# benattal/neural-radiance-caching

Measured on AMD Instinct MI355X. Metric: rays/sec (1024-ray batch, 64+64 proposal + 32 shaded samples/ray), hotdog cache forward, higher is better.
Workload: dtype f32

## Files before the change

neural-radiance-caching_amd/csrc/hostcheck.cpp:

```cpp
#include <stdio.h>
#include <stdlib.h>

#include <string>

#include "rc_pack_host.h"
#include "rc_ide_coef.h"
#include "rc_vis_plan.h"
#include "rc_ws.h"

using namespace rcpack;

static std::vector<float> read_f32(const std::string& path, size_t count) {
  std::vector<float> v(count);
  FILE* f = fopen(path.c_str(), "rb");
  if (!f || fread(v.data(), sizeof(float), count, f) != count) { fprintf(stderr, "hostcheck: cannot read %zu floats from %s\n", count, path.c_str()); exit(2); }
  fclose(f);
  return v;
}
static void write_f32(const std::string& path, const std::vector<float>& v) {
  FILE* f = fopen(path.c_str(), "wb");
  if (!f || fwrite(v.data(), sizeof(float), v.size(), f) != v.size()) { fprintf(stderr, "hostcheck: cannot write %s\n", path.c_str()); exit(2); }
  fclose(f);
}
static HostLayer layer(const std::string& dir, const char* name, int in, int out) {
// ... 23 lines not shown

static int transient_heads(const std::string& dir) {
  HostLayer slf = layer(dir, "slf", 128, 71), irr = layer(dir, "irr", 64, 70);
  write_f32(dir + "/out_tbins_split.bin", pack_bins_stream(slf, irr, 70, 192, true));
  write_f32(dir + "/out_tbins_f32.bin", pack_bins_stream(slf, irr, 70, 128, false));
  write_f32(dir + "/out_tslice_slf.bin", pack_slice_columns(slf, 4, 70, 132));
  write_f32(dir + "/out_tslice_irr.bin", pack_slice_columns(irr, 2, 70, 68));
  std::vector<float> v;
  for (float sigma : {3.0f, 4.0f, 0.7f, 0.0f}) {
    const std::vector<float> t = temporal_taps(sigma);
    v.push_back((float)t.size());
    v.insert(v.end(), t.begin(), t.end());
  }
  write_f32(dir + "/out_ttaps.bin", v);
  printf("hostcheck tbins ok\n");
  return 0;
}

template <size_t... K> static void emplace_kind(WsExtra& x, size_t kind, std::index_sequence<K...>) {
  ((kind == K ? (void)x.emplace<K>() : (void)0), ...);
}
static long ws_offset(WsBufs& s, const WsBuf* b) { return (long)((const char*)b - (const char*)&s); }
static int ws_registry(int num_levels, int n_names, char** names) {
  std::vector<WsBufs> sets(WS_COUNT);
  long lookups = 0;
  for (int id = 0; id < WS_COUNT; ++id) emplace_kind(sets[id].x, kWsSets[id].kind, std::make_index_sequence<std::variant_size_v<WsExtra>>());
  for (int id = 0; id < WS_COUNT; ++id) {
    WsBufs& s = sets[id];
    if (s.x.index() != kWsSets[id].kind) return 5;
    for (const WsName& e : wsn::kTable)
// ... 12 lines not shown
  for (int i = 0; i < n_names; ++i) {
    std::string leaf;
    const int id = ws_split(names[i], leaf);
    const WsBuf* b = id < 0 ? nullptr : ws_lookup(sets[id], leaf, num_levels);
    ++lookups;
    if (b) printf("probe %s %d %ld\n", names[i], id, ws_offset(sets[id], b));
    else printf("probe %s %d -\n", names[i], id);
  }
  size_t bufs = 0;
  for (int id = 0; id < WS_COUNT; ++id) ws_for_each(sets[id], [&](WsBuf& b) { bufs += b.p == nullptr; });
  printf("lookups %ld buffers %zu\nhostcheck ws ok\n", lookups, bufs);
  return 0;
}

int main(int argc, char** argv) {
  if (argc < 2) { fprintf(stderr, "usage: hostcheck <dir> | hostcheck --tbins <dir> | hostcheck --ide-inc | hostcheck --ws <num_levels> [name ...]\n"); return 2; }
  if (std::string(argv[1]) == "--ide-inc") return print_ide_inc();
  if (std::string(argv[1]) == "--tbins") {
    if (argc < 3) { fprintf(stderr, "usage: hostcheck --tbins <dir>\n"); return 2; }
    return transient_heads(argv[2]);
  }
  if (std::string(argv[1]) == "--ws") {
    if (argc < 3) { fprintf(stderr, "usage: hostcheck --ws <num_levels> [name ...]\n"); return 2; }
    return ws_registry(atoi(argv[2]), argc - 3, argv + 3);
  }
  const std::string dir = argv[1];
  {
    HostLayer L = layer(dir, "a", 37, 70);
    std::vector<Step> s;
    steps_natural(s, 37, 0); step_bias(s);
    write_f32(dir + "/out_pack.bin", pack(s, {tile_full(&L, 0), tile_full(&L, 1), tile_full(&L, 2)}));
  }
  {
    HostLayer L = layer(dir, "b", 64, 40);
    std::vector<Step> s;
// ... 88 lines not shown
```

neural-radiance-caching_amd/csrc/rc_api.hip:

```cpp
#include <dlfcn.h>
#include <math.h>
#include <stdlib.h>
#include <stdio.h>
#include <string.h>

#include <array>
#include <map>
#include <memory>
#include <string>
#include <variant>
#include <vector>

#include "rc_internal.h"
#include "rc_pack_host.h"
#include "rc_itof_host.h"
#include "rc_ws.h"
#include "rc_prng_host.h"

void rc_launch_hashgrid_src(const RcGridDev& g, const float* points, int soa_in, const int32_t* src, int64_t n_src,
                            int64_t n, float* out, int feature_major, int64_t ldo, float contract_radius,
                            float* jac_out, hipStream_t stream);
int rc_shader_lds_bytes();
int rc_weight_chunk_floats();
void rc_shader_prepare();
// ... 399 lines not shown
    if (hipStreamCreateWithPriority(&s, hipStreamNonBlocking, which == 0 ? prio_lo : prio_hi) != hipSuccess) s = nullptr;
  }
  return s;
}

int ensure_side_stream(rc_handle* h) {
  if (h->side_stream) return RC_OK;
  h->side_stream = rc_helper_stream(0);
  if (!h->side_stream) return fail(h, RC_ERR_HIP, "side stream");
  for (hipEvent_t& e : h->ev_side) RC_HIP(h, hipEventCreateWithFlags(&e, hipEventDisableTiming));
  return RC_OK;
}

int repack_transient(rc_handle* h);

int repack(rc_handle* h) {
  std::string missing;
  const rc_config& c = h->cfg;
  std::vector<float> fused_parts[4];
  if (!h->ide_table.p) {
    RcIdeTable tb;
    build_ide_table(tb);
    RC_HIP(h, hipMalloc((void**)&h->ide_table.p, sizeof(tb)));
    h->ide_table.bytes = sizeof(tb);
    RC_HIP(h, hipMemcpy(h->ide_table.p, &tb, sizeof(tb), hipMemcpyHostToDevice));
  }
  for (int g = 0; g < 4; ++g)
    for (size_t l = 0; l < h->grids[g].sizes.size(); ++l)
      if (!h->grids[g].loaded[l])
        return fail(h, RC_ERR_MISSING_WEIGHT,
                    "missing weight: " + h->grids[g].prefix + "/" + level_name(h->grids[g].cfg, h->grids[g].sizes, h->grids[g].sizes[l]));
  for (int l = 0; l < c.num_levels; ++l) {
    const std::string base = "params/Cache/Sampler/MLP_" + std::to_string(l);
    const HostLayer* d0 = need(h, base + "/density_layers_0", missing);
    const HostLayer* d1 = need(h, base + "/density_layers_1", missing);
    const HostLayer* dout = need(h, base + "/output_density_layer", missing);
    const HostLayer* dn = (l == c.num_levels - 1) ? need(h, base + "/pred_normals_layer", missing) : nullptr;
    if (!missing.empty()) return fail(h, RC_ERR_MISSING_WEIGHT, "missing weight: " + missing);
    std::vector<Step> s;
    steps_natural(s, d0->in, 0); step_bias(s);
    std::vector<float> stream = pack_f32(s, {tile_full(d0, 0), tile_full(d0, 1)});
    s.clear(); steps_acc(s, 2, 0); step_bias(s);
    append(stream, pack_f32(s, {tile_full(d1, 0), tile_full(d1, 1)}));
    std::vector<Col> regs = {Col{dout, 0}};
    if (dn) { regs.push_back(Col{dn, 0}); regs.push_back(Col{dn, 1}); regs.push_back(Col{dn, 2}); }
    append(stream, pack_dot(regs, 2, false));
    if (dn) {
      HostLayer w1t, w0t;
      w1t.in = d1->out; w1t.out = d1->in; w1t.kernel.resize(d1->kernel.size()); w1t.bias.assign(w1t.out, 0.0f);
      for (int r = 0; r < d1->in; ++r) for (int c2 = 0; c2 < d1->out; ++c2) w1t.kernel[(size_t)c2 * w1t.out + r] = d1->kernel[(size_t)r * d1->out + c2];
      w0t.in = d0->out; w0t.out = d0->in; w0t.kernel.resize(d0->kernel.size()); w0t.bias.assign(w0t.out, 0.0f);
      for (int r = 0; r < d0->in; ++r) for (int c2 = 0; c2 < d0->out; ++c2) w0t.kernel[(size_t)c2 * w0t.out + r] = d0->kernel[(size_t)r * d0->out + c2];
      std::vector<Step> sb; steps_acc(sb, 2, 0);
      append(stream, pack_f32(sb, {tile_full(&w1t, 0, 0, false), tile_full(&w1t, 1, 0, false)}));
      append(stream, pack_f32(sb, {tile_full(&w0t, 0, 0, false)}));
    }
    if (l < 3) fused_parts[l] = stream;
    int rc = upload(h, h->packs.dens[l], pad_stream(stream));
    if (rc) return rc;
  }
  if (h->transient) {
    int off[4];
    rc_fused_stream_offsets(&off[0], &off[1], &off[2], &off[3]);
    bool ok = fused_geometry_ok(h);
    std::vector<float> stream;
    for (int p = 0; p < 3 && ok; ++p) {
      ok = (int)(stream.size() / 64) == off[p];
      append(stream, fused_parts[p]);
    }
    if (ok && (int)(stream.size() / 64) < off[3] && off[3] - (int)(stream.size() / 64) < 4) stream.resize((size_t)off[3] * 64, 0.0f);
    ok = ok && (int)(stream.size() / 64) == off[3];
    h->fused_front_ok = ok;
    if (ok) {
      int rc = upload(h, h->packs.fused_front, pad_stream(stream));
      if (rc) return rc;
      if ((rc = build_fused_tables(h))) return rc;
    }
    return repack_transient(h);
  }
  const std::string sh = "params/Cache/Shader";
  const HostLayer* bott = need(h, sh + "/bottleneck_layer", missing);
  const HostLayer* rough = need(h, sh + "/roughness_layer", missing);
  const HostLayer* tint = need(h, sh + "/tint_layer", missing);
  const HostLayer* amb = need(h, sh + "/ambient_irradiance_layer", missing);
  const HostLayer* irr = need(h, sh + "/irradiance_layer", missing);
  const HostLayer* i0 = need(h, sh + "/integrated_brdf_layers_0", missing);
// ... 16 lines not shown
    for (int o = 0; o < lb->out; ++o) lbf.bias[o] = (float)((double)lbf.bias[o] + (double)lb->bias[o]);
    for (int o = 0; o < i0->out; ++o) i0f.bias[o] = (float)((double)i0f.bias[o] + (double)i0->bias[o]);
    steps_acc(s, 2, 0); steps_natural(s, 32, 64); step_bias(s);
    std::vector<Col> regs = {Col{rough, 0}, Col{tint, 0}, Col{tint, 1}, Col{tint, 2}, Col{amb, 0},
                             Col{amb, 1},   Col{amb, 2},  Col{irr, 0},  Col{irr, 1},  Col{irr, 2}};
    append(stream, pack(s, {tile_by_reg(regs)}));
    s.clear(); steps_acc(s, 2, 0); steps_natural(s, 32, 64);
    for (int i = 0; i < 36; ++i) s.push_back({{FE + i, FE + 36 + i}});
    step_bias(s);
    append(stream, pack(s, {tile_full(&l0f, 0), tile_full(&l0f, 1), tile_full(&l0f, 2), tile_full(&l0f, 3),
                            tile_full(&lbf, 0), tile_full(&lbf, 1), tile_full(&lbf, 2), tile_full(&lbf, 3)}));
    s.clear(); steps_acc(s, 2, 0); steps_natural(s, 32, 64); s.push_back({{FE, -2}});
    append(stream, pack(s, {tile_full(&i0f, 0), tile_full(&i0f, 1)}));
    s.clear(); steps_acc(s, 2, 0); step_bias(s);
    append(stream, pack(s, {tile_full(i1, 0), tile_full(i1, 1)}));
    append(stream, pack_dot({Col{io, 0}}, 2));
    s.clear(); steps_acc(s, 4, 0); step_bias(s);
    append(stream, pack(s, {tile_full(l1, 0), tile_full(l1, 1), tile_full(l1, 2), tile_full(l1, 3)}));
    append(stream, pack(s, {tile_full(l2, 0), tile_full(l2, 1), tile_full(l2, 2), tile_full(l2, 3)}));
    std::vector<Step> sb; steps_acc(sb, 4, 0);
    append(stream, pack(sb, {tile_full(lb, 0, 0, false), tile_full(lb, 1, 0, false), tile_full(lb, 2, 0, false),
                             tile_full(lb, 3, 0, false)}));
    append(stream, pack_dot({Col{la, 0}, Col{la, 1}, Col{la, 2}}, 4));
    fused_parts[3] = stream;
    int rc = upload(h, h->packs.shader, pad_stream(stream));
    if (rc) return rc;
  }
  {
    int off[4];
    const int nf = rc_fused_stream_offsets(&off[0], &off[1], &off[2], &off[3]);
    bool ok = fused_geometry_ok(h);
    std::vector<float> stream;
    for (int p = 0; p < 4 && ok; ++p) {
      if (p == 3 && (int)(stream.size() / 64) < off[p] && off[p] - (int)(stream.size() / 64) < 4) stream.resize((size_t)off[p] * 64, 0.0f);
      ok = (int)(stream.size() / 64) == off[p];
      append(stream, fused_parts[p]);
    }
    ok = ok && (int)(stream.size() / 64) == nf;
    h->fused_ok = ok;
    if (ok) {
      int rc = upload(h, h->packs.fused, pad_stream(stream));
      if (rc) return rc;
      if ((rc = build_fused_tables(h))) return rc;
    }
  }
  {
    std::string miss;
    const std::string ep = "params/Cache/EnvMap";
    const HostLayer* e0 = need(h, ep + "/layer_0", miss);
    const HostLayer* e1 = need(h, ep + "/layer_1", miss);
    const HostLayer* e2 = need(h, ep + "/layer_2", miss);
    const HostLayer* eb = need(h, ep + "/layer_bottleneck", miss);
    const HostLayer* eo = need(h, ep + "/output_rgba_layer", miss);
// ... 527 lines not shown
```

neural-radiance-caching_amd/csrc/rc_dev_mlp.h:

```cpp
#pragma once
#include "rc_internal.h"

namespace rcdev {

typedef float f32x16 __attribute__((ext_vector_type(16)));

constexpr int kWaves = 4;

__device__ __forceinline__ f32x16 zero16() {
  f32x16 z;
#pragma unroll
  for (int i = 0; i < 16; ++i) z[i] = 0.0f;
  return z;
}

typedef uint32_t u32x4 __attribute__((ext_vector_type(4)));
typedef __bf16 bf16x8 __attribute__((ext_vector_type(8)));

__device__ __forceinline__ uint32_t pack_top16(float a1, float a0) {
  return __builtin_amdgcn_perm(__float_as_uint(a1), __float_as_uint(a0), 0x07060302u);
}
__device__ __forceinline__ float top16(float a) { return __uint_as_float(__float_as_uint(a) & 0xffff0000u); }
typedef float f32x2 __attribute__((ext_vector_type(2)));
__device__ __forceinline__ f32x2 top16(f32x2 a) { return f32x2{top16(a[0]), top16(a[1])}; }
// ... 410 lines not shown
    for (int p = 0; p < PT; ++p) {
      float sum = part[p][o][0] + part[p][o][1];
      sum = sum + __shfl_xor(sum, 32, 64);
      out[p][o] = sum + bias;
    }
  }
}
template <int NT, int NO, int FBASE, int NF, bool KEEP = false, int W = kWaves, int NOB = NO, int CH = kChunk, class WS = WStream>
__device__ __forceinline__ void dot_out1(const WS& w, const f32x16 (&hid)[NT], float (&out)[NO],
                                         float (&keep)[KEEP ? NT * 16 : 1]) {
  const f32x16 (&h1)[1][NT] = reinterpret_cast<const f32x16 (&)[1][NT]>(hid);
  float (&o1)[1][NO] = reinterpret_cast<float (&)[1][NO]>(out);
  dot_out<1, NT, NO, FBASE, NF, KEEP, W, NOB, CH, WS>(w, h1, o1, keep);
}

__device__ __forceinline__ float softplus(float x) {
  return fmaxf(x, 0.0f) + log1pf(expf(-fabsf(x)));
}
__device__ __forceinline__ float sigmoidf(float x) { return 1.0f / (1.0f + expf(-x)); }
template <class F>
__device__ __forceinline__ void eval_pair(F f, int h, float xa, float xb, float& ya, float& yb) {
  const float y = f(h ? xb : xa);
  ya = y; yb = y;
  swap_halves(ya, yb);
}
__device__ __forceinline__ void softplus_pair(int h, float xa, float xb, float& ya, float& yb) {
  eval_pair([](float x) { return softplus(x); }, h, xa, xb, ya, yb);
}
__device__ __forceinline__ void sigmoid_pair(int h, float xa, float xb, float& ya, float& yb) {
  eval_pair([](float x) { return sigmoidf(x); }, h, xa, xb, ya, yb);
// ... 19 lines not shown
    if (v != v) return 0.0f;
    return fminf(fmaxf(v, -RC_FMAX), RC_FMAX);
  };
  x = fix(nx); y = fix(ny); z = fix(nz);
}


__host__ __device__ constexpr int ide_l(int i) { return i < 2 ? 1 : (i < 5 ? 2 : (i < 10 ? 4 : (i < 19 ? 8 : 16))); }
__host__ __device__ constexpr int ide_m(int i) { return i < 2 ? i : (i < 5 ? i - 2 : (i < 10 ? i - 5 : (i < 19 ? i - 10 : i - 19))); }


constexpr int kShActSteps = 102;
constexpr int kStepIde = 48;
constexpr int kStepBias = 84;

struct ShaderFrags {
  static constexpr int F_H = 0, F_S0 = F_H + rc_lfr(49, 1), F_I0 = F_S0 + rc_lfr(85, 8), F_I1 = F_I0 + rc_lfr(49, 2), F_IO = F_I1 + rc_lfr(33, 2),
                       F_S1 = F_IO + rc_dfr(1, 2), F_S2 = F_S1 + rc_lfr(65, 4), F_SB = F_S2 + rc_lfr(65, 4), F_SO = F_SB + rc_lfr(64, 4),
                       COUNT = F_SO + rc_dfr(3, 4);
};

struct ShaderConsts { float roughness_bias, irradiance_bias, ambient_bias, rgb_max, slf_ambient_bias; };
struct ShadeOut { float rgb[3], ad[3], idf[3], is[3], tint[3]; };

#ifdef RC_STAMPS
#define RC_TSTAMP(i) do { if (st) { __builtin_amdgcn_sched_barrier(0); st[i] = __builtin_amdgcn_s_memtime(); __builtin_amdgcn_sched_barrier(0); } } while (0)
#else
#define RC_TSTAMP(i) do { } while (0)
#endif
template <int F0, int NF, class WS = WStream>
__device__ __forceinline__ ShadeOut shader_tile(const WS& ws, float* act, int lane, int h, float nx, float ny, float nz,
                                                float vx, float vy, float vz, const ShaderConsts& k,
                                                unsigned long long* st = nullptr) {
  RC_TSTAMP(0);
  float rough, tint[3], ad[3], idf[3];
  float tint2_raw, idf2_raw;
  u32x4 fpc[6][3];
  if constexpr (kRcSplit) split_blocks<6>(act, fpc);
  {
    f32x16 acc[1];
    acc[0] = zero16();
    if constexpr (kRcSplit) mlp_layer_x<1, 49, F0 + ShaderFrags::F_H, NF, 6, true>(ws, act, acc, fpc);
    else mlp_layer<1, 49, F0 + ShaderFrags::F_H, NF>(ws, act, acc);
    float sp_ad[3], sp_idf[2];
    softplus_pair(h, acc[0][0] + k.roughness_bias, acc[0][4] + k.ambient_bias, rough, sp_ad[0]);
    softplus_pair(h, acc[0][5] + k.ambient_bias, acc[0][6] + k.ambient_bias, sp_ad[1], sp_ad[2]);
    softplus_pair(h, acc[0][7] + k.irradiance_bias, acc[0][8] + k.irradiance_bias, sp_idf[0], sp_idf[1]);
    sigmoid_pair(h, acc[0][1], acc[0][2], tint[0], tint[1]);
    tint2_raw = acc[0][3];
    idf2_raw = acc[0][9] + k.irradiance_bias;
#pragma unroll
    for (int c = 0; c < 3; ++c) ad[c] = fminf(fmaxf(sp_ad[c], 0.0f), k.rgb_max);
#pragma unroll
    for (int c = 0; c < 2; ++c) idf[c] = fminf(fmaxf(sp_idf[c], 0.0f), k.rgb_max);
  }
  RC_TSTAMP(1);
  float dot_nv;
  {
// ... 21 lines not shown
    for (int i = 0; i < RC_IDE_TERMS; ++i) {
      const int l = ide_l(i), m = ide_m(i);
      float poly = 0.0f;
#pragma unroll
      for (int k = 0; k < RC_IDE_ZPOW; ++k) {
        if (k <= l - m && ((l - m - k) & 1) == 0) poly = poly + zp[k] * kRcIdeCoef[i][k];
      }
      const float att = expf(-(0.5f * (float)(l * (l + 1))) * rough);
      act[(kStepIde + i) * 64] = (cpw[m] * poly) * att;
    }
  }
  RC_TSTAMP(2);
  f32x16 s0[8];
#pragma unroll
  for (int t = 0; t < 8; ++t) s0[t] = zero16();
  if constexpr (kRcSplit) mlp_layer_x<8, 85, F0 + ShaderFrags::F_S0, NF, 6, false>(ws, act, s0, fpc);
  else mlp_layer<8, 85, F0 + ShaderFrags::F_S0, NF>(ws, act, s0);
  RC_TSTAMP(3);
  float ibrdf;
  {
    f32x16 ib[2];
    ib[0] = zero16(); ib[1] = zero16();
    act[48 * 64] = h == 0 ? dot_nv : 1.0f;
    if constexpr (kRcSplit) mlp_layer_x<2, 49, F0 + ShaderFrags::F_I0, NF, 6, false>(ws, act, ib, fpc);
    else mlp_layer<2, 49, F0 + ShaderFrags::F_I0, NF>(ws, act, ib);
    BHand<2, true> hi;
    hand_off<2, true>(ib, lane, hi);
    ib[0] = zero16(); ib[1] = zero16();
    mlp_layer_h<2, 2, true, F0 + ShaderFrags::F_I1, NF>(ws, hi, ib);
    float o[1], nokeep[1];
    dot_out1<2, 1, F0 + ShaderFrags::F_IO, NF>(ws, ib, o, nokeep);
    sigmoid_pair(h, tint2_raw, o[0] + 1.0986123f, tint[2], ibrdf);
  }
  RC_TSTAMP(4);
  float amb[3];
  {
    f32x16 acc[4] = {s0[0], s0[1], s0[2], s0[3]};
    f32x16 skip[4] = {s0[4], s0[5], s0[6], s0[7]};
    BHand<4, true> hs;
    hand_off<4, true>(acc, lane, hs);
#pragma unroll
    for (int t = 0; t < 4; ++t) acc[t] = zero16();
    mlp_layer_h<4, 4, true, F0 + ShaderFrags::F_S1, NF>(ws, hs, acc);
    hand_off<4, true>(acc, lane, hs);
#pragma unroll
    for (int t = 0; t < 4; ++t) acc[t] = zero16();
    RC_TSTAMP(5);
    mlp_layer_h<4, 4, true, F0 + ShaderFrags::F_S2, NF>(ws, hs, acc);
    BHand<4, false> hb;
    hand_off<4, false>(acc, lane, hb);
    RC_TSTAMP(6);
    mlp_layer_h<4, 4, false, F0 + ShaderFrags::F_SB, NF>(ws, hb, skip);
    RC_TSTAMP(7);
    float o[3], nokeep[1];
    dot_out1<4, 3, F0 + ShaderFrags::F_SO, NF>(ws, skip, o, nokeep);
    float sp_idf2, sp_amb[3];
    softplus_pair(h, idf2_raw, o[0] + k.slf_ambient_bias, sp_idf2, sp_amb[0]);
    softplus_pair(h, o[1] + k.slf_ambient_bias, o[2] + k.slf_ambient_bias, sp_amb[1], sp_amb[2]);
    idf[2] = fminf(fmaxf(sp_idf2, 0.0f), k.rgb_max);
#pragma unroll
    for (int c = 0; c < 3; ++c) amb[c] = fmaxf(sp_amb[c], 0.0f);
  }
  RC_TSTAMP(8);
  ShadeOut o;
#pragma unroll
  for (int c = 0; c < 3; ++c) {
    const float is = fminf(fmaxf(tint[c] * ibrdf * (amb[c] * 1.0f), 0.0f), k.rgb_max);
    const float ambient = ad[c] + 0.0f;
    const float indirect = idf[c] + is;
    o.rgb[c] = ambient + indirect; o.ad[c] = ad[c]; o.idf[c] = idf[c]; o.is[c] = is; o.tint[c] = tint[c];
// ... 6 lines not shown
```

neural-radiance-caching_amd/csrc/rc_fused.hip:

```cpp
#include "rc_fused_common.h"
#include <type_traits>

using namespace rcdev;
using namespace rcfused;

namespace {

constexpr int kAppSteps = 32;

#define RC_OUT_PINS "s"(op[0]), "s"(op[1]), "s"(op[2]), "s"(op[3]), "s"(op[4]), "s"(op[5]), "s"(op[6]), "s"(op[7]), "s"(op[8]), "s"(op[9]), \
                    "s"(op[10]), "s"(op[11]), "s"(op[12]), "s"(op[13]), "s"(op[14]), "s"(op[15]), "s"(op[16]), "s"(op[17]), "s"(op[18])
#define RC_EXPORT_PINS "s"(a.f_tdist), "s"(a.f_density), "s"(a.f_means), "s"(a.f_normals_pred), "s"(a.n)

template <int K> struct LookupRegs { const float* table[K]; int32_t size[K]; uint32_t mask[K]; float bbox, precondition, contract_radius, density_bias; };
template <int K>
__device__ __forceinline__ LookupRegs<K> fetch_lookup(const RcLookupRec& q) {
  LookupRegs<K> g;
#pragma unroll
  for (int l = 0; l < K; ++l) { g.table[l] = q.table[l]; g.size[l] = q.size[l]; g.mask[l] = l < kFusedDense ? 0u : q.mask[l]; }
  g.bbox = q.bbox; g.precondition = q.precondition; g.contract_radius = q.contract_radius; g.density_bias = q.density_bias;
  return g;
}
#define RC_LOOKUP_PINS6(g) "s"(g.table[0]), "s"(g.table[1]), "s"(g.table[2]), "s"(g.table[3]), "s"(g.table[4]), "s"(g.table[5]),      \
                           "s"(g.size[0]), "s"(g.size[1]), "s"(g.size[2]), "s"(g.size[3]), "s"(g.size[4]), "s"(g.size[5]),              \
// ... 5 lines not shown
  static_assert(K >= 6 && K <= 8, "RC_LOOKUP_PINS6 and the levels behind it");
  if constexpr (K == 6) asm volatile("" :: RC_LOOKUP_PINS6(g));
  else if constexpr (K == 7) asm volatile("" :: RC_LOOKUP_PINS6(g), "s"(g.table[6]), "s"(g.size[6]), "s"(g.mask[6]));
  else asm volatile("" :: RC_LOOKUP_PINS6(g), "s"(g.table[6]), "s"(g.size[6]), "s"(g.mask[6]), "s"(g.table[7]), "s"(g.size[7]), "s"(g.mask[7]));
}
struct ShadeRegs { ShaderConsts sh; float bg; const float* lights; const float* viewdirs; float pct0, pct1, pct2; };
__device__ __forceinline__ ShadeRegs fetch_shade(const RcShadeRec& q) {
  return ShadeRegs{q.sh, q.bg, q.lights, q.viewdirs, q.pct[0], q.pct[1], q.pct[2]};
}
#define RC_SHADE_PINS(k) "s"(k.sh.roughness_bias), "s"(k.sh.irradiance_bias), "s"(k.sh.ambient_bias), "s"(k.sh.rgb_max), "s"(k.sh.slf_ambient_bias), \
                         "s"(k.bg), "s"(k.lights), "s"(k.viewdirs), "s"(k.pct0), "s"(k.pct1), "s"(k.pct2)

template <int K, int FB, int NF, class WS>
__device__ __forceinline__ float density_level64(const WS& ws, float* act_wave, int lane, const float (&f)[K]) {
  constexpr int KS0 = (K + 1) / 2 + 1;
  using FR = DensFrags<KS0>;
  const int tile = lane >> 5, j = lane & 31, h = lane >> 5;
#pragma unroll
  for (int k = 0; k < 2 * (KS0 - 1); ++k)
    act_wave[tile * kTileStride + (k >> 1) * 64 + j + 32 * (k & 1)] = k < K ? f[k < K ? k : 0] : 0.0f;
#pragma unroll
  for (int p = 0; p < 2; ++p) act_wave[p * kTileStride + (KS0 - 1) * 64 + lane] = h == 0 ? 1.0f : 0.0f;
  lds_sync<false>();
  float* act = act_wave + lane;
  f32x16 acc[2][2];
#pragma unroll
  for (int p = 0; p < 2; ++p) { acc[p][0] = zero16(); acc[p][1] = zero16(); }
  mlp_layer_pt<2, 2, KS0, FB + FR::D0, NF>(ws, act, kTileStride, acc);
  BHandPt<2, 2, true> hd;
#pragma unroll
  for (int p = 0; p < 2; ++p) hand_off<2, true>(acc[p], lane, hd.hand[p]);
#pragma unroll
  for (int p = 0; p < 2; ++p) { acc[p][0] = zero16(); acc[p][1] = zero16(); }
  mlp_layer_pth<2, 2, 2, true, FB + FR::D1, NF>(ws, hd, acc);
  float out[2][1], nokeep[1];
  dot_out<2, 2, 1, FB + FR::DO, NF>(ws, acc, out, nokeep);
  return tile == 0 ? out[0][0] : out[1][0];
}

template <int LEVEL, int K, int FB, int NF, class WS, class FETCH, class PIN>
__device__ __forceinline__ float proposal_level(const LookupRegs<K>& g, const WS& ws, float* act_wave, const Ray& r, const float* s_td, int lane,
                                                unsigned long long* stamps, const FETCH& fetch_next, const PIN& pin_next) {
  float mx, my, mz, t0, t1;
  mean_of(r, s_td, lane, mx, my, mz, t0, t1);
  float cx = mx, cy = my, cz = mz;
  contract3(cx, cy, cz, g.contract_radius);
  float f[K];
  {
    const float ux = unit_box(g.bbox, cx), uy = unit_box(g.bbox, cy), uz = unit_box(g.bbox, cz);
#if defined(RC_ABL) && RC_ABL == 11
    for (int l = 0; l < K; ++l) f[l] = ux * (float)l + uy - uz;
// ... 108 lines not shown
        const int l = half * 4 + q;
        float v[4], jd[GRAD ? 12 : 1];
        level2_combine<GRAD>(g2.precondition, C[q], v, jd);
#pragma unroll
        for (int c = 0; c < 4; ++c) f[4 * l + c] = v[c];
        if constexpr (GRAD) level2_jacobian(g2.precondition, g2.size[l], g2.bbox, l, jd, act_wave, j, h);
      }
    }
    const int base = h == 0 ? 0 : kAppSteps;
#pragma unroll
    for (int k = 0; k < 32; ++k) act_wave[(base + (k >> 1)) * 64 + j + 32 * (k & 1)] = f[k];
    act[16 * 64] = h == 0 ? 1.0f : 0.0f;
    lds_sync<false>();
  }
  RC_FSTAMP(8);
  using FR = DensFrags<17>;
  float density, npx, npy, npz, ngx = 0.0f, ngy = 0.0f, ngz = 0.0f;
  {
    f32x16 acc[2];
    acc[0] = zero16(); acc[1] = zero16();
    mlp_layer_d<2, 17, F_L2 + FR::D0, NF>(ws, act, acc);
    uint32_t m0 = 0, m1 = 0;
    if constexpr (GRAD) {
#pragma unroll
      for (int t = 0; t < 2; ++t)
#pragma unroll
        for (int r = 0; r < 16; ++r) m0 |= (acc[t][r] > 0.0f ? 1u : 0u) << (t * 16 + r);
    }
    {
      BHand<2, true> hd;
      hand_off<2, true>(acc, lane, hd);
      acc[0] = zero16(); acc[1] = zero16();
      mlp_layer_dh<2, 2, true, F_L2 + FR::D1, NF>(ws, hd, acc);
    }
    if constexpr (GRAD) {
#pragma unroll
      for (int t = 0; t < 2; ++t)
#pragma unroll
        for (int r = 0; r < 16; ++r) m1 |= (acc[t][r] > 0.0f ? 1u : 0u) << (t * 16 + r);
    }
    park<2, true>(acc, act, 0);
    float out[4], wout[GRAD ? 32 : 1];
    dot_out1<2, 4, F_L2 + FR::DO, NF, GRAD>(ws, acc, out, wout);
    if constexpr (!FRONT) asm volatile("" :: RC_SHADE_PINS(k));
    density = density_of(g2.density_bias, out[0], cx, cy, cz, g2.bbox);
    npx = out[1]; npy = out[2]; npz = out[3];
    neg_normalize(npx, npy, npz);
    if constexpr (GRAD) {
      BHand<2, false> bw;
      bw.one = 0.0f;
#pragma unroll
      for (int s = 0; s < 32; ++s) bw.v[s] = ((m1 >> s) & 1u) ? wout[s] : 0.0f;
      f32x16 g[2];
      g[0] = zero16(); g[1] = zero16();
      mlp_layer_dh<2, 2, false, F_L2 + FR::B1, NF>(ws, bw, g);
#pragma unroll
      for (int t = 0; t < 2; ++t)
#pragma unroll
// ... 15 lines not shown
      const int64_t np = a.n * 32, p = ray * 32 + j;
      export_samples<GRAD>(a, ray, lane, s.td, density, mx, my, mz, npx, npy, npz, ngx, ngy, ngz);
      float* hb = a.f_hbuf + ray * (32 * 64) + lane;
#pragma unroll
      for (int k = 0; k < 32; ++k) hb[k * 64] = act[k * 64];
#pragma unroll
      for (int k = 0; k < 16; ++k) a.f_app[(int64_t)(2 * k + h) * np + p] = act[(kAppSteps + k) * 64];
    }
    return;
  }
  act[48 * 64] = h == 0 ? 1.0f : 0.0f;
#if defined(RC_ABL) && RC_ABL == 12
  ShadeOut so;
  for (int c = 0; c < 3; ++c) { so.rgb[c] = act[c * 64]; so.ad[c] = npx; so.idf[c] = npy; so.is[c] = npz; so.tint[c] = density; }
#else
  const ShadeOut so = shader_tile<F_SH, NF>(ws, act, lane, h, npx, npy, npz, k.viewdirs[3 * ray], k.viewdirs[3 * ray + 1],
                                            k.viewdirs[3 * ray + 2], k.sh);
#endif

  RC_FSTAMP(10);
  const bool act_s = lane < 32;
  const float wnf = alpha_weight(density, t0, t1, r.dnorm, act_s, lane);
  constexpr int kOutPtrs = RC_OUT_LIGHT_DISTS + 1;
  float* op[kOutPtrs];
#pragma unroll
  for (int i = 0; i < kOutPtrs; ++i) op[i] = a.out.ptr[i];
  if constexpr (EXPORT) {
    asm volatile("" :: RC_EXPORT_PINS, RC_OUT_PINS);
  }
  __builtin_amdgcn_sched_barrier(0);
  if constexpr (EXPORT) {
// ... 161 lines not shown
```

neural-radiance-caching_amd/csrc/rc_fused_common.h:

```cpp
#pragma once
#include "rc_dev_grid.h"
#include "rc_dev_mlp.h"
#include "rc_dev_sample.h"

namespace rcfused {
using namespace rcdev;

constexpr int kTileStride = 33 * 64;
constexpr int kScratch = 7 * 68;
constexpr int kAppTmp = 33;
constexpr int kFusedDense = kRcFusedDenseLevels;
constexpr int kJac = 49;

template <int KS0> struct DensFrags {
  static constexpr int NO = KS0 == 17 ? 4 : 1;
  static constexpr int D0 = 0, D1 = rc_lfr32(KS0, 2), DO = D1 + rc_lfr32(33, 2), B1 = DO + rc_dfr32(NO, 2), B0 = B1 + rc_lfr32(32, 2), END = B0 + rc_lfr32(32, 1);
};
constexpr int F_L0 = 0;
constexpr int F_L1 = F_L0 + DensFrags<4>::B1;
constexpr int F_L2 = F_L1 + DensFrags<5>::B1;
constexpr int F_SH = rc_align_piece(F_L2 + DensFrags<17>::END);
constexpr int NF_FUSED = F_SH + ShaderFrags::COUNT;

#ifdef RC_STAMPS
#define RC_FSTAMP(i) do { __builtin_amdgcn_sched_barrier(0); __builtin_amdgcn_s_waitcnt(0); stamps[i] = __builtin_amdgcn_s_memtime(); __builtin_amdgcn_sched_barrier(0); } while (0)
#else
#define RC_FSTAMP(i) do { } while (0)
#endif

#ifdef RC_STAMPS
#define RC_FSTAMP_NOWAIT(i) do { __builtin_amdgcn_sched_barrier(0); stamps[i] = __builtin_amdgcn_s_memtime(); __builtin_amdgcn_sched_barrier(0); } while (0)
#else
#define RC_FSTAMP_NOWAIT(i) do { } while (0)
#endif
#ifdef RC_STAMPS
#define RC_FSTAMP_BUF stamps
#else
// ... 199 lines not shown
```

neural-radiance-caching_amd/csrc/rc_pack_host.h:

```cpp
#pragma once
#include <math.h>
#include <stdint.h>
#include <string.h>

#include <array>
#include <vector>

#ifndef RC_IDE_TERMS
#define RC_IDE_TERMS 36
#define RC_IDE_ZPOW 17
struct RcIdeTable {
  float coef[RC_IDE_TERMS][RC_IDE_ZPOW];
  int32_t m[RC_IDE_TERMS];
  float sigma[RC_IDE_TERMS];
};
#endif

#if defined(__HIPCC__)
#define RC_HD __host__ __device__
#else
#define RC_HD
#endif

RC_HD inline bool rc_cell_corner(int N, int64_t i, int64_t* entry) {
// ... 16 lines not shown
#ifndef RC_SPLIT_MFMA
#define RC_SPLIT_MFMA 1
#endif
constexpr bool kRcSplit = RC_SPLIT_MFMA != 0;
#if !RC_SPLIT_MFMA || defined(RC_TEAM_SPLIT_DIAG)
#define RC_TEAM_KERNEL 1
#else
#define RC_TEAM_KERNEL 0
#endif
constexpr int rc_lfr(int ks, int nt) { return kRcSplit ? ((ks + 7) / 8) * nt * 12 : ks * nt; }
constexpr int rc_dfr(int no, int nt) { return kRcSplit ? ((no * (nt * 16 + 1) + 3) / 4) * 4 : no * (nt * 16 + 1); }
constexpr int rc_lfr32(int ks, int nt) { return ks * nt; }
constexpr int rc_dfr32(int no, int nt) { return no * (nt * 16 + 1); }
constexpr int rc_align_piece(int f) { return kRcSplit ? (f + 3) / 4 * 4 : f; }

namespace rcpack {

struct HostLayer {
  std::vector<float> kernel, bias;
  int in = 0, out = 0;
  bool have_kernel = false, have_bias = false;
};

struct Step { int row[2]; };
struct Col {
  const HostLayer* L = nullptr;
  int col = 0;
  int row_off = 0;
  bool bias_ok = true;
};
// ... 27 lines not shown
  return tl;
}

inline std::vector<float> pack_dot(const std::vector<Col>& outs, int ntiles, bool pad_to_piece = kRcSplit) {
  std::vector<float> v;
  for (const Col& c : outs)
    for (int t = 0; t < ntiles; ++t)
      for (int r = 0; r < 16; ++r)
        for (int lane = 0; lane < 64; ++lane) {
          const int row = acc_feat(t, r, lane >> 5) + c.row_off;
          v.push_back((c.L && row < c.L->in) ? c.L->kernel[(size_t)row * c.L->out + c.col] : 0.0f);
        }
  for (const Col& c : outs)
    for (int lane = 0; lane < 64; ++lane) v.push_back(c.L ? c.L->bias[c.col] : 0.0f);
  if (pad_to_piece) v.resize((size_t)rc_dfr((int)outs.size(), ntiles) * 64, 0.0f);
  return v;
}

inline float pack_value(const Step& st, int h, const Col& c) {
  if (!c.L) return 0.0f;
  const int row = st.row[h];
  if (row == -2) return c.bias_ok ? c.L->bias[c.col] : 0.0f;
  if (row >= 0) {
    const int rr = row + c.row_off;
    if (rr < c.L->in) return c.L->kernel[(size_t)rr * c.L->out + c.col];
  }
  return 0.0f;
}

inline void split3(float x, uint16_t (&piece)[3]) {
// ... 142 lines not shown
```

Measured before the change: 10.42 million.

## Pack fused output dot weights as compact per-half row tables

Adds a compact row-table layout for the small output dot products in the fused kernel. Each half-wave reads its weights as contiguous f32x4 vectors instead of one float per lane per fragment, and the bias is stored once instead of per lane. The fragment offsets for the density levels and the shader are recomputed, with alignment so that each table sits inside one ring chunk. This shrinks the streamed weight bytes and the per-lane load count, but adds padding and a new host packing path.

```diff
diff --git a/neural-radiance-caching_amd/csrc/hostcheck.cpp b/neural-radiance-caching_amd/csrc/hostcheck.cpp
--- a/neural-radiance-caching_amd/csrc/hostcheck.cpp
+++ b/neural-radiance-caching_amd/csrc/hostcheck.cpp
@@ -61,6 +61,39 @@
   }
   write_f32(dir + "/out_ttaps.bin", v);
   printf("hostcheck tbins ok\n");
+  return 0;
+}
+
+template <bool ROWS> static void print_fused() {
+  using namespace rcfused;
+  using F = FusedFrags<ROWS>;
+  using SF = rcdev::ShaderFragsL<ROWS, F::SH>;
+  printf("fused rows=%d F_L0=%d F_L1=%d F_L2=%d F_SH=%d NF_FUSED=%d chunks=%d\n", (int)ROWS, F::L0, F::L1, F::L2, F::SH, F::NF,
+         (F::NF + kRcChunkFrags - 1) / kRcChunkFrags);
+  printf("dens rows=%d DO0=%d DO1=%d DO2=%d B1_2=%d END2=%d\n", (int)ROWS, F::L0 + DensFrags<4, ROWS, F::L0>::DO,
+         F::L1 + DensFrags<5, ROWS, F::L1>::DO, F::L2 + DensFrags<17, ROWS, F::L2>::DO, F::L2 + DensFrags<17, ROWS, F::L2>::B1,
+         F::L2 + DensFrags<17, ROWS, F::L2>::END);
+  printf("shader rows=%d F_H=%d F_S0=%d F_I0=%d F_I1=%d F_IO=%d F_S1=%d F_S2=%d F_SB=%d F_SO=%d COUNT=%d\n", (int)ROWS, SF::F_H, SF::F_S0,
+         SF::F_I0, SF::F_I1, SF::F_IO, SF::F_S1, SF::F_S2, SF::F_SB, SF::F_SO, SF::COUNT);
+}
+static int output_rows(const std::string& dir) {
+  if (dir.empty()) {
+    print_fused<false>();
+    print_fused<true>();
+    printf("layout rows=%d NF_FUSED=%d\n", (int)kRcFusedRows, rcfused::NF_FUSED);
+    return 0;
+  }
+  HostLayer L = layer(dir, "d", 64, 3);
+  const std::vector<Col> outs = {Col{&L, 0}, Col{&L, 1}, Col{&L, 2}};
+  write_f32(dir + "/out_rows.bin", pack_dot_rows(outs, 2, false));
+  write_f32(dir + "/out_rows_piece.bin", pack_dot_rows(outs, 2, true));
+  write_f32(dir + "/out_rows_dot.bin", pack_dot(outs, 2, false));
+  printf("rows split=%d stride=%d floats=%d frags=%d piece_frags=%d\n", (int)kRcSplit, rc_rows_stride(3, 2), rc_rows_floats(3, 2),
+         rc_rfr(3, 2, false), rc_rfr(3, 2, true));
+  print_fused<false>();
+  print_fused<true>();
+  printf("layout rows=%d NF_FUSED=%d\n", (int)kRcFusedRows, rcfused::NF_FUSED);
+  printf("hostcheck rows ok\n");
   return 0;
 }
 
@@ -103,11 +136,14 @@
 }
 
 int main(int argc, char** argv) {
-  if (argc < 2) { fprintf(stderr, "usage: hostcheck <dir> | hostcheck --tbins <dir> | hostcheck --ide-inc | hostcheck --ws <num_levels> [name ...]\n"); return 2; }
+  if (argc < 2) { fprintf(stderr, "usage: hostcheck <dir> | hostcheck --tbins <dir> | hostcheck --rows <dir> | hostcheck --ide-inc | hostcheck --ws <num_levels> [name ...]\n"); return 2; }
   if (std::string(argv[1]) == "--ide-inc") return print_ide_inc();
   if (std::string(argv[1]) == "--tbins") {
     if (argc < 3) { fprintf(stderr, "usage: hostcheck --tbins <dir>\n"); return 2; }
     return transient_heads(argv[2]);
+  }
+  if (std::string(argv[1]) == "--rows") {
+    return output_rows(argc < 3 ? "" : argv[2]);
   }
   if (std::string(argv[1]) == "--ws") {
     if (argc < 3) { fprintf(stderr, "usage: hostcheck --ws <num_levels> [name ...]\n"); return 2; }
diff --git a/neural-radiance-caching_amd/csrc/rc_api.hip b/neural-radiance-caching_amd/csrc/rc_api.hip
--- a/neural-radiance-caching_amd/csrc/rc_api.hip
+++ b/neural-radiance-caching_amd/csrc/rc_api.hip
@@ -437,10 +437,45 @@
 
 int repack_transient(rc_handle* h);
 
+struct FusedParts {
+  std::vector<float> head[3], tail[3];
+  std::vector<Col> rows[3];
+  std::vector<float> sh_head, sh_trunk;
+  std::vector<Col> io, so;
+};
+bool put_at(std::vector<float>& stream, int at, const std::vector<float>& v, int max_gap) {
+  const int have = (int)(stream.size() / 64);
+  if (stream.size() % 64 != 0 || have > at || at - have > max_gap) return false;
+  stream.resize((size_t)at * 64, 0.0f);
+  append(stream, v);
+  return true;
+}
+std::vector<float> fused_dot(const std::vector<Col>& outs, int ntiles, bool pad_to_piece) {
+  return kRcFusedRows ? pack_dot_rows(outs, ntiles, pad_to_piece) : pack_dot(outs, ntiles, pad_to_piece);
+}
+bool build_fused_stream(const FusedParts& P, bool with_shader, std::vector<float>& stream) {
+  using namespace rcfused;
+  const int row_gap = kRcFusedRows ? kRcChunkFrags - 1 : 0;
+  bool ok = true;
+  auto level = [&](int l, int fb, int d_o, int b1) {
+    ok = ok && put_at(stream, fb, P.head[l], 0) && put_at(stream, fb + d_o, fused_dot(P.rows[l], 2, false), row_gap) &&
+         put_at(stream, fb + b1, P.tail[l], 0);
+  };
+  level(0, F_L0, FusedDens<4, F_L0>::DO, FusedDens<4, F_L0>::B1);
+  level(1, F_L1, FusedDens<5, F_L1>::DO, FusedDens<5, F_L1>::B1);
+  level(2, F_L2, FusedDens<17, F_L2>::DO, FusedDens<17, F_L2>::B1);
+  ok = ok && put_at(stream, F_SH, {}, 3);
+  if (!with_shader) return ok;
+  using SF = FusedShader;
+  ok = ok && put_at(stream, F_SH + SF::F_H, P.sh_head, 0) && put_at(stream, F_SH + SF::F_IO, fused_dot(P.io, 2, kRcSplit), row_gap) &&
+       put_at(stream, F_SH + SF::F_S1, P.sh_trunk, 0) && put_at(stream, F_SH + SF::F_SO, fused_dot(P.so, 4, kRcSplit), row_gap);
+  return ok && (int)(stream.size() / 64) == NF_FUSED;
+}
+
 int repack(rc_handle* h) {
   std::string missing;
   const rc_config& c = h->cfg;
-  std::vector<float> fused_parts[4];
+  FusedParts fused_parts;
   if (!h->ide_table.p) {
     RcIdeTable tb;
     build_ide_table(tb);
@@ -467,7 +502,9 @@
     append(stream, pack_f32(s, {tile_full(d1, 0), tile_full(d1, 1)}));
     std::vector<Col> regs = {Col{dout, 0}};
     if (dn) { regs.push_back(Col{dn, 0}); regs.push_back(Col{dn, 1}); regs.push_back(Col{dn, 2}); }
+    if (l < 3) { fused_parts.head[l] = stream; fused_parts.rows[l] = regs; }
     append(stream, pack_dot(regs, 2, false));
+    const size_t tail_at = stream.size();
     if (dn) {
       HostLayer w1t, w0t;
       w1t.in = d1->out; w1t.out = d1->in; w1t.kernel.resize(d1->kernel.size()); w1t.bias.assign(w1t.out, 0.0f);
@@ -478,21 +515,15 @@
       append(stream, pack_f32(sb, {tile_full(&w1t, 0, 0, false), tile_full(&w1t, 1, 0, false)}));
       append(stream, pack_f32(sb, {tile_full(&w0t, 0, 0, false)}));
     }
-    if (l < 3) fused_parts[l] = stream;
+    if (l < 3) fused_parts.tail[l].assign(stream.begin() + tail_at, stream.end());
     int rc = upload(h, h->packs.dens[l], pad_stream(stream));
     if (rc) return rc;
   }
   if (h->transient) {
     int off[4];
     rc_fused_stream_offsets(&off[0], &off[1], &off[2], &off[3]);
-    bool ok = fused_geometry_ok(h);
     std::vector<float> stream;
-    for (int p = 0; p < 3 && ok; ++p) {
-      ok = (int)(stream.size() / 64) == off[p];
-      append(stream, fused_parts[p]);
-    }
-    if (ok && (int)(stream.size() / 64) < off[3] && off[3] - (int)(stream.size() / 64) < 4) stream.resize((size_t)off[3] * 64, 0.0f);
-    ok = ok && (int)(stream.size() / 64) == off[3];
+    const bool ok = fused_geometry_ok(h) && off[3] == rcfused::F_SH && build_fused_stream(fused_parts, false, stream);
     h->fused_front_ok = ok;
     if (ok) {
       int rc = upload(h, h->packs.fused_front, pad_stream(stream));
@@ -539,29 +570,27 @@
     append(stream, pack(s, {tile_full(&i0f, 0), tile_full(&i0f, 1)}));
     s.clear(); steps_acc(s, 2, 0); step_bias(s);
     append(stream, pack(s, {tile_full(i1, 0), tile_full(i1, 1)}));
-    append(stream, pack_dot({Col{io, 0}}, 2));
+    fused_parts.sh_head = stream;
+    fused_parts.io = {Col{io, 0}};
+    append(stream, pack_dot(fused_parts.io, 2));
+    const size_t trunk_at = stream.size();
     s.clear(); steps_acc(s, 4, 0); step_bias(s);
     append(stream, pack(s, {tile_full(l1, 0), tile_full(l1, 1), tile_full(l1, 2), tile_full(l1, 3)}));
     append(stream, pack(s, {tile_full(l2, 0), tile_full(l2, 1), tile_full(l2, 2), tile_full(l2, 3)}));
     std::vector<Step> sb; steps_acc(sb, 4, 0);
     append(stream, pack(sb, {tile_full(lb, 0, 0, false), tile_full(lb, 1, 0, false), tile_full(lb, 2, 0, false),
                              tile_full(lb, 3, 0, false)}));
-    append(stream, pack_dot({Col{la, 0}, Col{la, 1}, Col{la, 2}}, 4));
-    fused_parts[3] = stream;
+    fused_parts.sh_trunk.assign(stream.begin() + trunk_at, stream.end());
+    fused_parts.so = {Col{la, 0}, Col{la, 1}, Col{la, 2}};
+    append(stream, pack_dot(fused_parts.so, 4));
     int rc = upload(h, h->packs.shader, pad_stream(stream));
     if (rc) return rc;
   }
   {
     int off[4];
     const int nf = rc_fused_stream_offsets(&off[0], &off[1], &off[2], &off[3]);
-    bool ok = fused_geometry_ok(h);
     std::vector<float> stream;
-    for (int p = 0; p < 4 && ok; ++p) {
-      if (p == 3 && (int)(stream.size() / 64) < off[p] && off[p] - (int)(stream.size() / 64) < 4) stream.resize((size_t)off[p] * 64, 0.0f);
-      ok = (int)(stream.size() / 64) == off[p];
-      append(stream, fused_parts[p]);
-    }
-    ok = ok && (int)(stream.size() / 64) == nf;
+    const bool ok = fused_geometry_ok(h) && nf == rcfused::NF_FUSED && build_fused_stream(fused_parts, true, stream);
     h->fused_ok = ok;
     if (ok) {
       int rc = upload(h, h->packs.fused, pad_stream(stream));
diff --git a/neural-radiance-caching_amd/csrc/rc_dev_mlp.h b/neural-radiance-caching_amd/csrc/rc_dev_mlp.h
--- a/neural-radiance-caching_amd/csrc/rc_dev_mlp.h
+++ b/neural-radiance-caching_amd/csrc/rc_dev_mlp.h
@@ -448,6 +448,61 @@
   dot_out<1, NT, NO, FBASE, NF, KEEP, W, NOB, CH, WS>(w, h1, o1, keep);
 }
 
+template <int PT, int NT, int NO, int FBASE, int NF, bool KEEP = false, int W = kWaves, int NOB = NO, int CH = kChunk, class WS = WStream>
+__device__ __forceinline__ void dot_rows(const WS& w, const f32x16 (&hid)[PT][NT], float (&out)[PT][NO],
+                                         float (&keep)[KEEP ? NT * 16 : 1]) {
+  constexpr int N = NOB * NT * 16, S = rc_rows_stride(NOB, NT), NFR = rc_rfr(NOB, NT, false);
+  static_assert(CH == kRcChunkFrags, "rc_rows_at places the block by the ring's chunk");
+  static_assert(FBASE / CH == (FBASE + NFR - 1) / CH, "a row table lies in one chunk of the ring");
+  static_assert(FBASE + NFR <= NF, "inside the stream");
+  if (FBASE > 0 && FBASE % CH == 0) ws_advance<NF, W, CH>(w, FBASE / CH);
+  const float* row = w.ring + (FBASE % (2 * CH)) * 64 + (w.lane >> 5) * S;
+  const float* bias = w.ring + (FBASE % (2 * CH)) * 64 + S + N;
+  float part[PT][NO][2];
+#pragma unroll
+  for (int p = 0; p < PT; ++p)
+#pragma unroll
+    for (int o = 0; o < NO; ++o) { part[p][o][0] = 0.0f; part[p][o][1] = 0.0f; }
+#pragma unroll
+  for (int o = 0; o < NO; ++o)
+#pragma unroll
+    for (int t = 0; t < NT; ++t)
+#pragma unroll
+      for (int r4 = 0; r4 < 4; ++r4) {
+        const f32x4 wv4 = *reinterpret_cast<const f32x4*>(row + (o * NT + t) * 16 + 4 * r4);
+#pragma unroll
+        for (int i = 0; i < 4; ++i) {
+          const int r = 4 * r4 + i;
+          const float wv = wv4[i];
+          if constexpr (KEEP) { if (o == 0) keep[t * 16 + r] = wv; }
+#pragma unroll
+          for (int p = 0; p < PT; ++p) part[p][o][r & 1] = __builtin_fmaf(relu0(hid[p][t][r]), wv, part[p][o][r & 1]);
+        }
+      }
+#pragma unroll
+  for (int o = 0; o < NO; ++o) {
+    const float b = bias[o];
+#pragma unroll
+    for (int p = 0; p < PT; ++p) {
+      float sum = part[p][o][0] + part[p][o][1];
+      sum = sum + __shfl_xor(sum, 32, 64);
+      out[p][o] = sum + b;
+    }
+  }
+}
+template <int NT, int NO, int FBASE, int NF, bool KEEP = false, int W = kWaves, int NOB = NO, int CH = kChunk, class WS = WStream>
+__device__ __forceinline__ void dot_rows1(const WS& w, const f32x16 (&hid)[NT], float (&out)[NO],
+                                          float (&keep)[KEEP ? NT * 16 : 1]) {
+  const f32x16 (&h1)[1][NT] = reinterpret_cast<const f32x16 (&)[1][NT]>(hid);
+  float (&o1)[1][NO] = reinterpret_cast<float (&)[1][NO]>(out);
+  dot_rows<1, NT, NO, FBASE, NF, KEEP, W, NOB, CH, WS>(w, h1, o1, keep);
+}
+template <class SF, int NT, int NO, int FBASE, int NF, class WS>
+__device__ __forceinline__ void dot_out_sf(const WS& w, const f32x16 (&hid)[NT], float (&out)[NO], float (&keep)[1]) {
+  if constexpr (SF::kRows) dot_rows1<NT, NO, FBASE, NF, false, kWaves, NO, kChunk, WS>(w, hid, out, keep);
+  else dot_out1<NT, NO, FBASE, NF, false, kWaves, NO, kChunk, WS>(w, hid, out, keep);
+}
+
 __device__ __forceinline__ float softplus(float x) {
   return fmaxf(x, 0.0f) + log1pf(expf(-fabsf(x)));
 }
@@ -497,11 +552,6 @@
 constexpr int kStepIde = 48;
 constexpr int kStepBias = 84;
 
-struct ShaderFrags {
-  static constexpr int F_H = 0, F_S0 = F_H + rc_lfr(49, 1), F_I0 = F_S0 + rc_lfr(85, 8), F_I1 = F_I0 + rc_lfr(49, 2), F_IO = F_I1 + rc_lfr(33, 2),
-                       F_S1 = F_IO + rc_dfr(1, 2), F_S2 = F_S1 + rc_lfr(65, 4), F_SB = F_S2 + rc_lfr(65, 4), F_SO = F_SB + rc_lfr(64, 4),
-                       COUNT = F_SO + rc_dfr(3, 4);
-};
 
 struct ShaderConsts { float roughness_bias, irradiance_bias, ambient_bias, rgb_max, slf_ambient_bias; };
 struct ShadeOut { float rgb[3], ad[3], idf[3], is[3], tint[3]; };
@@ -511,7 +561,7 @@
 #else
 #define RC_TSTAMP(i) do { } while (0)
 #endif
-template <int F0, int NF, class WS = WStream>
+template <int F0, int NF, class WS = WStream, class SF = ShaderFrags>
 __device__ __forceinline__ ShadeOut shader_tile(const WS& ws, float* act, int lane, int h, float nx, float ny, float nz,
                                                 float vx, float vy, float vz, const ShaderConsts& k,
                                                 unsigned long long* st = nullptr) {
@@ -523,8 +573,8 @@
   {
     f32x16 acc[1];
     acc[0] = zero16();
-    if constexpr (kRcSplit) mlp_layer_x<1, 49, F0 + ShaderFrags::F_H, NF, 6, true>(ws, act, acc, fpc);
-    else mlp_layer<1, 49, F0 + ShaderFrags::F_H, NF>(ws, act, acc);
+    if constexpr (kRcSplit) mlp_layer_x<1, 49, F0 + SF::F_H, NF, 6, true>(ws, act, acc, fpc);
+    else mlp_layer<1, 49, F0 + SF::F_H, NF>(ws, act, acc);
     float sp_ad[3], sp_idf[2];
     softplus_pair(h, acc[0][0] + k.roughness_bias, acc[0][4] + k.ambient_bias, rough, sp_ad[0]);
     softplus_pair(h, acc[0][5] + k.ambient_bias, acc[0][6] + k.ambient_bias, sp_ad[1], sp_ad[2]);
@@ -576,22 +626,22 @@
   f32x16 s0[8];
 #pragma unroll
   for (int t = 0; t < 8; ++t) s0[t] = zero16();
-  if constexpr (kRcSplit) mlp_layer_x<8, 85, F0 + ShaderFrags::F_S0, NF, 6, false>(ws, act, s0, fpc);
-  else mlp_layer<8, 85, F0 + ShaderFrags::F_S0, NF>(ws, act, s0);
+  if constexpr (kRcSplit) mlp_layer_x<8, 85, F0 + SF::F_S0, NF, 6, false>(ws, act, s0, fpc);
+  else mlp_layer<8, 85, F0 + SF::F_S0, NF>(ws, act, s0);
   RC_TSTAMP(3);
   float ibrdf;
   {
     f32x16 ib[2];
     ib[0] = zero16(); ib[1] = zero16();
     act[48 * 64] = h == 0 ? dot_nv : 1.0f;
-    if constexpr (kRcSplit) mlp_layer_x<2, 49, F0 + ShaderFrags::F_I0, NF, 6, false>(ws, act, ib, fpc);
-    else mlp_layer<2, 49, F0 + ShaderFrags::F_I0, NF>(ws, act, ib);
+    if constexpr (kRcSplit) mlp_layer_x<2, 49, F0 + SF::F_I0, NF, 6, false>(ws, act, ib, fpc);
+    else mlp_layer<2, 49, F0 + SF::F_I0, NF>(ws, act, ib);
     BHand<2, true> hi;
     hand_off<2, true>(ib, lane, hi);
     ib[0] = zero16(); ib[1] = zero16();
-    mlp_layer_h<2, 2, true, F0 + ShaderFrags::F_I1, NF>(ws, hi, ib);
+    mlp_layer_h<2, 2, true, F0 + SF::F_I1, NF>(ws, hi, ib);
     float o[1], nokeep[1];
-    dot_out1<2, 1, F0 + ShaderFrags::F_IO, NF>(ws, ib, o, nokeep);
+    dot_out_sf<SF, 2, 1, F0 + SF::F_IO, NF>(ws, ib, o, nokeep);
     sigmoid_pair(h, tint2_raw, o[0] + 1.0986123f, tint[2], ibrdf);
   }
   RC_TSTAMP(4);
@@ -603,19 +653,19 @@
     hand_off<4, true>(acc, lane, hs);
 #pragma unroll
     for (int t = 0; t < 4; ++t) acc[t] = zero16();
-    mlp_layer_h<4, 4, true, F0 + ShaderFrags::F_S1, NF>(ws, hs, acc);
+    mlp_layer_h<4, 4, true, F0 + SF::F_S1, NF>(ws, hs, acc);
     hand_off<4, true>(acc, lane, hs);
 #pragma unroll
     for (int t = 0; t < 4; ++t) acc[t] = zero16();
     RC_TSTAMP(5);
-    mlp_layer_h<4, 4, true, F0 + ShaderFrags::F_S2, NF>(ws, hs, acc);
+    mlp_layer_h<4, 4, true, F0 + SF::F_S2, NF>(ws, hs, acc);
     BHand<4, false> hb;
     hand_off<4, false>(acc, lane, hb);
     RC_TSTAMP(6);
-    mlp_layer_h<4, 4, false, F0 + ShaderFrags::F_SB, NF>(ws, hb, skip);
+    mlp_layer_h<4, 4, false, F0 + SF::F_SB, NF>(ws, hb, skip);
     RC_TSTAMP(7);
     float o[3], nokeep[1];
-    dot_out1<4, 3, F0 + ShaderFrags::F_SO, NF>(ws, skip, o, nokeep);
+    dot_out_sf<SF, 4, 3, F0 + SF::F_SO, NF>(ws, skip, o, nokeep);
     float sp_idf2, sp_amb[3];
     softplus_pair(h, idf2_raw, o[0] + k.slf_ambient_bias, sp_idf2, sp_amb[0]);
     softplus_pair(h, o[1] + k.slf_ambient_bias, o[2] + k.slf_ambient_bias, sp_amb[1], sp_amb[2]);
diff --git a/neural-radiance-caching_amd/csrc/rc_fused.hip b/neural-radiance-caching_amd/csrc/rc_fused.hip
--- a/neural-radiance-caching_amd/csrc/rc_fused.hip
+++ b/neural-radiance-caching_amd/csrc/rc_fused.hip
@@ -43,7 +43,7 @@
 template <int K, int FB, int NF, class WS>
 __device__ __forceinline__ float density_level64(const WS& ws, float* act_wave, int lane, const float (&f)[K]) {
   constexpr int KS0 = (K + 1) / 2 + 1;
-  using FR = DensFrags<KS0>;
+  using FR = FusedDens<KS0, FB>;
   const int tile = lane >> 5, j = lane & 31, h = lane >> 5;
 #pragma unroll
   for (int k = 0; k < 2 * (KS0 - 1); ++k)
@@ -63,7 +63,8 @@
   for (int p = 0; p < 2; ++p) { acc[p][0] = zero16(); acc[p][1] = zero16(); }
   mlp_layer_pth<2, 2, 2, true, FB + FR::D1, NF>(ws, hd, acc);
   float out[2][1], nokeep[1];
-  dot_out<2, 2, 1, FB + FR::DO, NF>(ws, acc, out, nokeep);
+  if constexpr (kRcFusedRows) dot_rows<2, 2, 1, FB + FR::DO, NF>(ws, acc, out, nokeep);
+  else dot_out<2, 2, 1, FB + FR::DO, NF>(ws, acc, out, nokeep);
   return tile == 0 ? out[0][0] : out[1][0];
 }
 
@@ -202,7 +203,7 @@
     lds_sync<false>();
   }
   RC_FSTAMP(8);
-  using FR = DensFrags<17>;
+  using FR = FusedDens<17, F_L2>;
   float density, npx, npy, npz, ngx = 0.0f, ngy = 0.0f, ngz = 0.0f;
   {
     f32x16 acc[2];
@@ -229,7 +230,8 @@
     }
     park<2, true>(acc, act, 0);
     float out[4], wout[GRAD ? 32 : 1];
-    dot_out1<2, 4, F_L2 + FR::DO, NF, GRAD>(ws, acc, out, wout);
+    if constexpr (kRcFusedRows) dot_rows1<2, 4, F_L2 + FR::DO, NF, GRAD>(ws, acc, out, wout);
+    else dot_out1<2, 4, F_L2 + FR::DO, NF, GRAD>(ws, acc, out, wout);
     if constexpr (!FRONT) asm volatile("" :: RC_SHADE_PINS(k));
     density = density_of(g2.density_bias, out[0], cx, cy, cz, g2.bbox);
     npx = out[1]; npy = out[2]; npz = out[3];
@@ -275,7 +277,7 @@
   ShadeOut so;
   for (int c = 0; c < 3; ++c) { so.rgb[c] = act[c * 64]; so.ad[c] = npx; so.idf[c] = npy; so.is[c] = npz; so.tint[c] = density; }
 #else
-  const ShadeOut so = shader_tile<F_SH, NF>(ws, act, lane, h, npx, npy, npz, k.viewdirs[3 * ray], k.viewdirs[3 * ray + 1],
+  const ShadeOut so = shader_tile<F_SH, NF_FUSED, WStream, FusedShader>(ws, act, lane, h, npx, npy, npz, k.viewdirs[3 * ray], k.viewdirs[3 * ray + 1],
                                             k.viewdirs[3 * ray + 2], k.sh);
 #endif
 
diff --git a/neural-radiance-caching_amd/csrc/rc_fused_common.h b/neural-radiance-caching_amd/csrc/rc_fused_common.h
--- a/neural-radiance-caching_amd/csrc/rc_fused_common.h
+++ b/neural-radiance-caching_amd/csrc/rc_fused_common.h
@@ -12,15 +12,7 @@
 constexpr int kFusedDense = kRcFusedDenseLevels;
 constexpr int kJac = 49;
 
-template <int KS0> struct DensFrags {
-  static constexpr int NO = KS0 == 17 ? 4 : 1;
-  static constexpr int D0 = 0, D1 = rc_lfr32(KS0, 2), DO = D1 + rc_lfr32(33, 2), B1 = DO + rc_dfr32(NO, 2), B0 = B1 + rc_lfr32(32, 2), END = B0 + rc_lfr32(32, 1);
-};
-constexpr int F_L0 = 0;
-constexpr int F_L1 = F_L0 + DensFrags<4>::B1;
-constexpr int F_L2 = F_L1 + DensFrags<5>::B1;
-constexpr int F_SH = rc_align_piece(F_L2 + DensFrags<17>::END);
-constexpr int NF_FUSED = F_SH + ShaderFrags::COUNT;
+static_assert(kChunk == kRcChunkFrags, "rc_rows_at places the row tables by the ring's chunk");
 
 #ifdef RC_STAMPS
 #define RC_FSTAMP(i) do { __builtin_amdgcn_sched_barrier(0); __builtin_amdgcn_s_waitcnt(0); stamps[i] = __builtin_amdgcn_s_memtime(); __builtin_amdgcn_sched_barrier(0); } while (0)
diff --git a/neural-radiance-caching_amd/csrc/rc_pack_host.h b/neural-radiance-caching_amd/csrc/rc_pack_host.h
--- a/neural-radiance-caching_amd/csrc/rc_pack_host.h
+++ b/neural-radiance-caching_amd/csrc/rc_pack_host.h
@@ -54,6 +54,50 @@
 constexpr int rc_dfr32(int no, int nt) { return no * (nt * 16 + 1); }
 constexpr int rc_align_piece(int f) { return kRcSplit ? (f + 3) / 4 * 4 : f; }
 
+constexpr int kRcChunkFrags = 64;
+constexpr bool kRcFusedRows = kRcSplit && !RC_TEAM_KERNEL;
+constexpr int rc_rows_stride(int no, int nt) { return (no * nt * 16 + 31) / 32 * 32 + (((no * nt * 16 + 31) / 32) % 2 == 0 ? 32 : 0); }
+constexpr int rc_rows_floats(int no, int nt) { return rc_rows_stride(no, nt) + no * nt * 16 + no; }
+constexpr int rc_rfr(int no, int nt, bool piece) { return piece ? (rc_rows_floats(no, nt) + 255) / 256 * 4 : (rc_rows_floats(no, nt) + 63) / 64; }
+constexpr int rc_rows_at(int f, int nfr) {
+  return f / kRcChunkFrags != (f + nfr - 1) / kRcChunkFrags ? (f + kRcChunkFrags - 1) / kRcChunkFrags * kRcChunkFrags : f;
+}
+
+namespace rcdev {
+template <bool ROWS, int F0 = 0>
+struct ShaderFragsL {
+  static constexpr bool kRows = ROWS;
+  static constexpr int F_H = 0, F_S0 = F_H + rc_lfr(49, 1), F_I0 = F_S0 + rc_lfr(85, 8), F_I1 = F_I0 + rc_lfr(49, 2),
+                       F_IO = ROWS ? rc_rows_at(F0 + F_I1 + rc_lfr(33, 2), rc_rfr(1, 2, kRcSplit)) - F0 : F_I1 + rc_lfr(33, 2),
+                       F_S1 = F_IO + (ROWS ? rc_rfr(1, 2, kRcSplit) : rc_dfr(1, 2)), F_S2 = F_S1 + rc_lfr(65, 4), F_SB = F_S2 + rc_lfr(65, 4),
+                       F_SO = ROWS ? rc_rows_at(F0 + F_SB + rc_lfr(64, 4), rc_rfr(3, 4, kRcSplit)) - F0 : F_SB + rc_lfr(64, 4),
+                       COUNT = F_SO + (ROWS ? rc_rfr(3, 4, kRcSplit) : rc_dfr(3, 4));
+  static_assert((F0 + F_S1) % 4 == 0 || !kRcSplit, "the layer behind a row table starts on a whole piece");
+};
+using ShaderFrags = ShaderFragsL<false>;
+}
+
+namespace rcfused {
+template <int KS0, bool ROWS = false, int FB = 0> struct DensFrags {
+  static constexpr int NO = KS0 == 17 ? 4 : 1;
+  static constexpr int D0 = 0, D1 = rc_lfr32(KS0, 2),
+                       DO = ROWS ? rc_rows_at(FB + D1 + rc_lfr32(33, 2), rc_rfr(NO, 2, false)) - FB : D1 + rc_lfr32(33, 2),
+                       B1 = DO + (ROWS ? rc_rfr(NO, 2, false) : rc_dfr32(NO, 2)), B0 = B1 + rc_lfr32(32, 2), END = B0 + rc_lfr32(32, 1);
+};
+template <bool ROWS> struct FusedFrags {
+  static constexpr int L0 = 0;
+  static constexpr int L1 = L0 + DensFrags<4, ROWS, L0>::B1;
+  static constexpr int L2 = L1 + DensFrags<5, ROWS, L1>::B1;
+  static constexpr int SH = rc_align_piece(L2 + DensFrags<17, ROWS, L2>::END);
+  static constexpr int NF = SH + rcdev::ShaderFragsL<ROWS, SH>::COUNT;
+  static_assert(SH % 4 == 0 || !kRcSplit, "F_SH: the shader's split layers start on a whole 1-KiB piece");
+};
+constexpr int F_L0 = FusedFrags<kRcFusedRows>::L0, F_L1 = FusedFrags<kRcFusedRows>::L1, F_L2 = FusedFrags<kRcFusedRows>::L2,
+              F_SH = FusedFrags<kRcFusedRows>::SH, NF_FUSED = FusedFrags<kRcFusedRows>::NF;
+template <int KS0, int FB> using FusedDens = DensFrags<KS0, kRcFusedRows, FB>;
+using FusedShader = rcdev::ShaderFragsL<kRcFusedRows, F_SH>;
+}
+
 namespace rcpack {
 
 struct HostLayer {
@@ -111,6 +155,21 @@
   for (const Col& c : outs)
     for (int lane = 0; lane < 64; ++lane) v.push_back(c.L ? c.L->bias[c.col] : 0.0f);
   if (pad_to_piece) v.resize((size_t)rc_dfr((int)outs.size(), ntiles) * 64, 0.0f);
+  return v;
+}
+
+inline std::vector<float> pack_dot_rows(const std::vector<Col>& outs, int ntiles, bool pad_to_piece = kRcSplit) {
+  const int no = (int)outs.size(), n = no * ntiles * 16, stride = rc_rows_stride(no, ntiles);
+  std::vector<float> v((size_t)rc_rfr(no, ntiles, pad_to_piece) * 64, 0.0f);
+  for (int h = 0; h < 2; ++h)
+    for (int o = 0; o < no; ++o)
+      for (int t = 0; t < ntiles; ++t)
+        for (int r = 0; r < 16; ++r) {
+          const Col& c = outs[o];
+          const int row = acc_feat(t, r, h) + c.row_off;
+          v[(size_t)h * stride + (o * ntiles + t) * 16 + r] = (c.L && row < c.L->in) ? c.L->kernel[(size_t)row * c.L->out + c.col] : 0.0f;
+        }
+  for (int o = 0; o < no; ++o) v[(size_t)stride + n + o] = outs[o].L ? outs[o].L->bias[outs[o].col] : 0.0f;
   return v;
 }
 
```

After: 10.64 million, median of 6. +2.0%, better.
